# LemonATsu/UNet-PhaseGen

Measured on AMD Instinct MI355X. Metric: spectrogram-frames/sec (train fwd+bwd), higher is better.
Workload: dtype f32; 1 GPU; train.py full step (fwd + cos/sin/mag loss + bwd + Adam), UNetModel(1024, 2048), per-GPU batch 64 x 1024 bins x 256 frames (BASELINE configs[2]); global_batch=64, frames=256, channels=1024, parallelism=dp1, grad_allreduce_payload=fp32, adam=fused into the wgrad epilogues

## Files before the change

### include/phasegen.h

```cpp
#ifndef PHASEGEN_H
#define PHASEGEN_H
#include <stdint.h>

#ifdef __cplusplus
extern "C" {
#endif

#define PG_VERSION 400

enum { PG_OK = 0, PG_ERR_NULL = -1, PG_ERR_SHAPE = -2, PG_ERR_ALIGN = -3, PG_ERR_UNSUPPORTED = -4,
       PG_ERR_WORKSPACE = -5 };

enum { PG_ACT_NONE = 0, PG_ACT_LEAKY02 = 1 , PG_ACT_RELU = 2  };

struct pg_adam_args;
typedef struct pg_conv_args {
    int32_t B, Cin, Cout, Lin, Lout, k, stride, pad;
    const float* x;  int64_t x_bs;
    int32_t x_act;
    int32_t precision;
    const float* w;
    float* y;        int64_t y_bs;
    const float* dy; int64_t dy_bs;
    float* dx;       int64_t dx_bs;
    const float* dx_add; int64_t dx_add_bs;
    const float* dx_ref; int64_t dx_ref_bs;
    int32_t dx_mask;
    int32_t schedule;
    float* dw;
    int32_t y_act; int32_t y2_act;
    float* y2;       int64_t y2_bs;
    void* workspace; int64_t workspace_bytes;
    const struct pg_adam_args* adam;
} pg_conv_args;
int64_t pg_workspace_bytes_conv(void);
int64_t pg_workspace_bytes_wgrad(const pg_conv_args* a, int32_t op);
enum { PG_PREC_FP32 = 0, PG_PREC_BF16 = 1, PG_PREC_BF16X3 = 2 };
enum { PG_SCHED_AUTO = 0, PG_SCHED_TILE_PER_WG = 1, PG_SCHED_FORCE_STREAMK = 2, PG_SCHED_NO_RAW = 4, PG_SCHED_NO_TALL = 8,
       PG_SCHED_CONTENDED = 16, PG_SCHED_NO_PS = 128, PG_SCHED_NO_RAW3 = 0x2000, PG_SCHED_ALL_RAW3 = 0x4000, PG_SCHED_NO_COLSPLIT = 0x20000, PG_SCHED_COLSPLIT = 0x40000 };
#define PG_SCHED_OVERSUB(f) (((f) & 15) << 8)

int pg_conv1d_fwd(const pg_conv_args* a, void* stream);
int pg_conv1d_dgrad(const pg_conv_args* a, void* stream);
int pg_conv1d_wgrad(const pg_conv_args* a, void* stream);
int pg_convt1d_fwd(const pg_conv_args* a, void* stream);
int pg_convt1d_dgrad(const pg_conv_args* a, void* stream);
int pg_convt1d_wgrad(const pg_conv_args* a, void* stream);
enum { PG_OP_CONV1D_FWD = 0, PG_OP_CONV1D_DGRAD = 1, PG_OP_CONV1D_WGRAD = 2,
       PG_OP_CONVT1D_FWD = 3, PG_OP_CONVT1D_DGRAD = 4, PG_OP_CONVT1D_WGRAD = 5 };
int pg_conv_describe(const pg_conv_args* a, int32_t op, char* buf, int32_t buflen);

#define PG_H_HEAD 32
typedef struct pg_convh_args {
    int32_t B, Cin, Cout, Lin, Lout, k, stride, pad;
    int32_t transposed;
    int32_t schedule;
    const uint16_t* x; int64_t x_bs;
    int32_t x_pitch; int32_t _pad0;
    const uint16_t* w;
    float* y; int64_t y_bs;
    uint16_t* yh; int64_t yh_bs; int32_t yh_pitch; int32_t yh_act;
    uint16_t* yh2; int64_t yh2_bs; int32_t yh2_pitch; int32_t yh2_act;
    void* workspace; int64_t workspace_bytes;
} pg_convh_args;
int pg_conv_fwd_h(const pg_convh_args* a, void* stream);
int pg_conv_fwd_h_supported(const pg_convh_args* a);
int pg_conv_fwd_h_describe(const pg_convh_args* a, char* buf, int32_t buflen);
int64_t pg_shadow_elems(int32_t Cin, int32_t Cout, int32_t k, int32_t stride, int32_t transposed);
int pg_shadow_weights(const float* w, uint16_t* wh, int32_t Cin, int32_t Cout, int32_t k, int32_t stride, int32_t transposed, void* stream);
typedef struct pg_cast_args { int32_t B, C, L, pitch, act, _pad0; const float* x; int64_t x_bs; uint16_t* y; int64_t y_bs; } pg_cast_args;
int pg_cast_rows_bf16(const pg_cast_args* a, void* stream);

typedef struct pg_bn_args {
    int32_t B, C, L; float eps, momentum;
    const float* x;  int64_t x_bs;
    float* y;        int64_t y_bs;
    const float* gamma; const float* beta;
    float* save_mean; float* save_invstd;
    float* running_mean; float* running_var;
    const float* dy; int64_t dy_bs;
    float* dx;       int64_t dx_bs;
    float* dgamma; float* dbeta;
    int32_t y_act; int32_t y2_act;
    float* y2;       int64_t y2_bs;
    uint16_t* yh;  int64_t yh_bs;  int32_t yh_pitch;  int32_t yh_act;
    uint16_t* yh2; int64_t yh2_bs; int32_t yh2_pitch; int32_t yh2_act;
    int64_t* num_batches_tracked;
} pg_bn_args;
int pg_bn_fwd(const pg_bn_args* a, void* stream);
int pg_bn_bwd(const pg_bn_args* a, void* stream);

typedef struct pg_clipnorm_args {
// ... 144 lines not shown
```

### unet-phasegen_amd/csrc/conv_common.h

```cpp
#pragma once
#include <hip/hip_runtime.h>
#include <stdint.h>
#include "phasegen.h"
#include "pg_common.h"

namespace pgconv {

struct IgemmParams {
    const float* x; long x_bs;
    const float* w;
    const float* pt; long pt_bs;
    float* y; long y_bs;
    const float* add; long add_bs;
    const float* ref; long ref_bs;
    unsigned x_bytes, w_bytes, pt_bytes;
    int B, Q, M, Lx, Ly, k, s, p;
    int act_x, act_p, mask_mode;
    int U, u_off;
    int LP; float inv_LP;
    int a_vec;
    int tilesM, tilesN;
    int g_ps;
    int tn_stride;
    float* y2; long y2_bs; float y_slope, y2_slope;
    float* ws;
    int nslab;
    int whole;
    int sr;
    int n_lo;
    int x_pitch;
    unsigned short* yh; long yh_bs; int yh_pitch; float yh_slope;
    unsigned short* yh2; long yh2_bs; int yh2_pitch; float yh2_slope;
    float* ad_p; float* ad_m; float* ad_v; PgAdamScalars ad;
    const float* qk; unsigned qk_bytes; int qk_bs, Lq;
    const float* pk; unsigned pk_bytes; int Kp;
};

}
using pgconv::IgemmParams;

namespace {


constexpr int WMB = 4;
constexpr int BM = 64 * WMB, BN = 128, BK = 16, NT = 256;
constexpr int TILE_A = BM * BK, TILE_B = BN * BK;
constexpr int STAGE = TILE_A + TILE_B;
constexpr int AE = BM / 16;

typedef float f32x16 __attribute__((ext_vector_type(16)));


typedef __amdgpu_buffer_rsrc_t rsrc_t;
constexpr int OOB = 0x7ffffff0;
__device__ __forceinline__ rsrc_t make_rsrc(const float* p, unsigned bytes) {
    return __builtin_amdgcn_make_buffer_rsrc(const_cast<float*>(p), 0, (int)bytes, 0x00020000);
}
__device__ __forceinline__ float bload(rsrc_t r, int elem_off, bool ok) {
    return __builtin_bit_cast(float, __builtin_amdgcn_raw_buffer_load_b32(r, ok ? elem_off * 4 : OOB, 0, 0));
}

__device__ __forceinline__ int xcd_remap(int bid, int nwg) {
    const int xcd = bid & 7, local = bid >> 3, q = nwg >> 3, r = nwg & 7;
    return (xcd < r ? xcd * (q + 1) : r * (q + 1) + (xcd - r) * q) + local;
}

template <int MB, int NB> struct AccT { f32x16 c[MB][NB]; };
using Acc = AccT<WMB, 2>;
using AccR = AccT<2, 4>;

__device__ __forceinline__ int dma_kt(int lane, int w) { return ((((lane >> 2) & 3) ^ w) << 2) | (lane & 3); }
__device__ __forceinline__ int dma_row(int lane, int w, int e) { return 16 * e + 4 * w + (lane >> 4); }

__device__ __forceinline__ int dma16_row(int lane, int w, int e) { return (4 * e + w) * 16 + (lane >> 2); }
__device__ __forceinline__ int dma16_kc(int lane) { return ((lane & 3) ^ ((lane >> 4) & 3)) << 2; }
#ifndef PG_ABL
#define PG_ABL 0
#endif
#if PG_ABL == 4
#define PG_ADDR(x) ((x) & 0x3f0)
#else
#define PG_ADDR(x) (x)
#endif
__device__ __forceinline__ void dma16(rsrc_t r, float* lds_wave_uniform, int byte_off) {
    __builtin_amdgcn_raw_ptr_buffer_load_lds(r, lds_wave_uniform, 16, PG_ADDR(byte_off), 0, 0, 0);
}
__device__ __forceinline__ void dma4(rsrc_t r, float* lds_wave_uniform, int byte_off) {
    __builtin_amdgcn_raw_ptr_buffer_load_lds(r, lds_wave_uniform, 4, PG_ADDR(byte_off), 0, 0, 0);
// ... 325 lines not shown
#pragma unroll
        for (int i = 0; i < MB; ++i)
#pragma unroll
            for (int q = 0; q < 2; ++q) {
                const int mb = m0 + wm * (MB * 32) + i * 32 + 16 * q + 4 * (lane >> 5);
                float pp[8], mm[8], vv[8];
#pragma unroll
                for (int r = 0; r < 8; ++r) {
                    const int m = mb + (r & 3) + 8 * (r >> 2);
                    const unsigned o = (unsigned)(m < p.M ? m : 0) * (unsigned)Ntot + (unsigned)n;
                    pp[r] = p.ad_p[o]; mm[r] = p.ad_m[o]; vv[r] = p.ad_v[o];
                }
#pragma unroll
                for (int r = 0; r < 8; ++r) {
                    const int m = mb + (r & 3) + 8 * (r >> 2);
                    if (m >= p.M) continue;
                    const unsigned o = (unsigned)m * (unsigned)Ntot + (unsigned)n;
                    pg_adam_one(pp[r], acc.c[i][j][8 * q + r], mm[r], vv[r], p.ad.omb1, p.ad.b2, p.ad.omb2, p.ad.step_size, p.ad.bc2_sqrt,
                                p.ad.eps, p.ad.gs);
                    p.ad_p[o] = pp[r]; p.ad_m[o] = mm[r]; p.ad_v[o] = vv[r];
                }
                __builtin_amdgcn_sched_barrier(0);
            }
    }
}

constexpr int NEVER = 0x40000000;
constexpr int FAR = (int)0x80000000u;


#if PG_ABL == 7
#define PG_STAMP(i) { unsigned long long t_; asm volatile("s_memtime %0\n\ts_waitcnt lgkmcnt(0)" : "=s"(t_) :: "memory"); \
                      __builtin_amdgcn_sched_barrier(0); if (i) st_sum[i - 1] += t_ - st_prev; st_prev = t_; }
#define PG_STAMP_FLUSH if (lane == 0) { for (int i_ = 0; i_ < 3; ++i_) atomicAdd((unsigned long long*)p.ws + i_, st_sum[i_]); \
                                        atomicAdd((unsigned long long*)p.ws + 3, (unsigned long long)(se - sb)); }
#define PG_STAMP_DECL unsigned long long st_sum[3] = {0, 0, 0}, st_prev = 0;
#else
#define PG_STAMP(i)
#define PG_STAMP_FLUSH
#define PG_STAMP_DECL
#endif

__device__ __forceinline__ void divmod24(int n, int d, float inv, int& q, int& r) {
    q = (int)((float)n * inv);
    r = n - q * d;
    if (r < 0) { r += d; --q; }
    if (r >= d) { r -= d; ++q; }
}

constexpr int RBM = 128, RBN = 256;
constexpr int RS2 = 768, RS1 = 384;
constexpr int raw_gap(int tj) { return tj >= 8 ? 16 : tj; }
constexpr int RTILE_A = RBM * BK;
constexpr int g_wlp(int kw, int s) { return kw == 32 ? 64 : (kw == 8 ? (s == 1 ? 24 : 40) : 36); }

inline bool unet_ks(int k, int s) { return (k == 32 && s == 2) || (k == 8 && s == 1) || (k == 8 && s == 2) || (k == 4 && s == 2) || (k == 5 && s == 2); }

enum Kind { KIND_F, KIND_T, KIND_G };

}

namespace pgconv {
hipError_t launch_im2col(int kind, const IgemmParams& p, int grid, hipStream_t st, int prec);
hipError_t launch_raw_ft(int kind, const IgemmParams& p, int grid, hipStream_t st, int prec);
hipError_t launch_raw_ft_tall(int kind, const IgemmParams& p, int grid, hipStream_t st, int prec);
hipError_t launch_raw_g(const IgemmParams& p, int grid, hipStream_t st, int prec);
hipError_t launch_h3(int kind, const IgemmParams& p, int grid, hipStream_t st);
bool raw3_covers(int kind, const IgemmParams& p);
hipError_t launch_raw3(int kind, const IgemmParams& p, int grid, hipStream_t st);
bool h_supported(int kind, const IgemmParams& p);
}
```

### unet-phasegen_amd/csrc/conv_igemm.hip

```cpp
#include <hip/hip_runtime.h>
#include <cstring>
#include <cmath>
#include <algorithm>
#include "conv_fixup.h"

namespace {

constexpr int WG_PER_CU = 2;
constexpr int MAX_STREAMK_WG = 2048;
constexpr long WS_PER_WG = 2L * ACC_REGS * NT * 4;
constexpr long WS_STREAMK = (long)MAX_STREAMK_WG * WS_PER_WG;

struct Knobs {
    int prec;
    int force_mode;
    int no_raw;
    int no_tall;
    int oversub;
    int contended;
    int no_ps;
    int no_raw3;
    int all_raw3;
    int sr;
    int force_colsplit;
    int no_colsplit;
};
int decode_knobs(const pg_conv_args* a, Knobs& k) {
    if (a->precision < 0 || a->precision > 2) return pg_fail(PG_ERR_UNSUPPORTED, "conv: precision must be PG_PREC_FP32, PG_PREC_BF16 or PG_PREC_BF16X3");
    const int sc = a->schedule;
    if (sc < 0 || (sc & ~0x7ffff) || ((sc >> 17) & 3) == 3 || (sc & 3) == 3 || ((sc >> 8) & 15) > 8) return pg_fail(PG_ERR_SHAPE, "conv: bad schedule bits");
    k.prec = a->precision;
    k.force_mode = sc & 3; k.no_raw = (sc >> 2) & 1; k.no_tall = (sc >> 3) & 1;
    k.oversub = (sc >> 8) & 15; if (!k.oversub) k.oversub = 4;
    k.contended = (sc >> 4) & 1;
    if ((sc >> 5) & 3) return pg_fail(PG_ERR_UNSUPPORTED, "conv: schedule bits 5-6 (tile families removed in 0.4)");
    k.no_ps = (sc >> 7) & 1;
    k.no_raw3 = (sc >> 13) & 1;
    k.all_raw3 = (sc >> 14) & 1;
    k.sr = ((sc >> 15) & 3) ? 1 << (((sc >> 15) & 3) - 1) : 0;
    k.no_colsplit = (sc >> 17) & 1;
    k.force_colsplit = (sc >> 18) & 1;
    if (k.no_raw3 && k.all_raw3) return pg_fail(PG_ERR_SHAPE, "conv: schedule bits 13 and 14 exclude each other");
    return PG_OK;
}

bool fixup_wide(int grid, long split_tiles) { return split_tiles > 0 && grid >= 8 * split_tiles; }

int pick_grid(long tiles, int nslab, IgemmParams& p, long ws_bytes, const Knobs& kn, bool one_wave) {
    const long total = tiles * (long)nslab;
    const long slots = (long)pg_cu_count() * (one_wave ? 1 : WG_PER_CU), ws_per_wg = one_wave ? 2 * WS_PER_WG : WS_PER_WG;
    ws_bytes = std::min(ws_bytes, WS_STREAMK);
    p.whole = 0;
    if (kn.force_mode == 0 && !kn.contended && tiles % slots == 0) {
        if (tiles <= slots * kn.oversub) return (int)tiles;
        for (long mult = kn.oversub; mult >= 1; --mult)
            if (tiles % (slots * mult) == 0) return (int)(slots * mult);
    }
    long mult = total / (256 * slots);
    if (mult > kn.oversub) mult = kn.oversub;
    if (mult < 1) mult = 1;
    long G = slots * mult;
    if (G > MAX_STREAMK_WG) G = (MAX_STREAMK_WG / slots) * slots;
    if (G > total) G = total;
    const bool can = p.ws && ws_bytes >= G * ws_per_wg && total < 0x7fffffffL;
    if (kn.force_mode == 1 || !can) return (int)tiles;
    if (kn.force_mode == 2) return (int)G;
    if (!kn.contended && tiles > slots) {
        const long whole = tiles / slots * slots, rem = tiles - whole;
        if (rem * nslab >= slots * 8 && whole + slots <= MAX_STREAMK_WG && ws_bytes >= (whole + slots) * ws_per_wg) {
            p.whole = (int)whole;
            return (int)(whole + slots);
        }
    }
    return total >= slots * 8 ? (int)G : (int)tiles;
}

bool raw_supported(Kind kind, const IgemmParams& p, const Knobs& kn, int tn = RBN) {
    if (kn.no_raw || !unet_ks(p.k, p.s) || (kind == KIND_F && p.k == 5 && p.Q % 2)) return false;
    if (kind == KIND_G) return p.LP >= 16;
    const bool t = kind == KIND_T;
    const int kv = p.k == 5 ? 8 : p.k, kwp = t ? kv / p.s : kv, sc = t ? 1 : p.s, lcol = t ? p.U : p.Ly;
    const int tj = kwp < 16 ? kwp : 16;
    const int nseg_max = (lcol - 1 + tn - 1) / lcol + 1;
    return sc * (tn - 1) + tj + raw_gap(tj) * (nseg_max - 1) + (t ? tj : 0) <= (sc == 1 ? RS1 : RS2);
}

long g_pack_layout(IgemmParams& p) {
    const int cps = (p.LP + 15) / 16;
    const long gimax = p.g_ps ? 16L * (cps - 1) : (long)p.LP - 1;
    long lq = (long)p.s * gimax + g_wlp(p.k, p.s);
    if (lq < (long)p.p + p.Lx) lq = (long)p.p + p.Lx;
    lq = (lq + 3) / 4 * 4;
    const long kp = p.g_ps ? 16L * cps : 16L * p.nslab;
    const long qbytes = (long)p.B * p.Q * lq * 4, pbytes = (p.g_ps ? (long)p.B : 1L) * p.M * kp * 4;
// ... 127 lines not shown
struct ConvOp { Kind kind; bool tr, swap; const char* null_msg; };
const ConvOp CONV_OPS[6] = {
    {KIND_F, false, false, "conv1d_fwd: x, w, y required"},
    {KIND_T, false, true, "conv1d_dgrad: dy, w, dx required"},
    {KIND_G, false, false, "conv1d_wgrad: dy, x, dw required"},
    {KIND_T, true, false, "convt1d_fwd: x, w, y required"},
    {KIND_F, true, true, "convt1d_dgrad: dy, w, dx required"},
    {KIND_G, true, true, "convt1d_wgrad: dy, x, dw required"}};

int plan_conv(int op, const pg_conv_args* a, bool ptrs, ConvPlan& pl) {
    const ConvOp& o = CONV_OPS[op];
    if (int e = check_geom(a, o.tr)) return e;
    Knobs kn; if (int e = decode_knobs(a, kn)) return e;
    IgemmParams p = {};
    p.B = a->B; p.k = a->k; p.s = a->stride; p.p = a->pad;
    p.M = o.swap ? a->Cin : a->Cout; p.Q = o.swap ? a->Cout : a->Cin; p.Lx = o.swap ? a->Lout : a->Lin;
    const int lo = o.swap ? a->Lin : a->Lout;
    p.x = o.swap ? a->dy : a->x; p.x_bs = o.swap ? a->dy_bs : a->x_bs; p.act_x = o.swap ? PG_ACT_NONE : a->x_act;
    if (o.kind == KIND_G) {
        p.pt = o.swap ? a->x : a->dy; p.pt_bs = o.swap ? a->x_bs : a->dy_bs; p.act_p = o.swap ? a->x_act : PG_ACT_NONE;
        p.LP = lo; p.y = a->dw;
    } else if (o.swap) {
        p.w = a->w; p.Ly = lo; p.y = a->dx; p.y_bs = a->dx_bs; p.y_slope = 1.0f; p.y2_slope = 1.0f;
        p.add = a->dx_add; p.add_bs = a->dx_add_bs; p.ref = a->dx_ref; p.ref_bs = a->dx_ref_bs;
        p.mask_mode = a->dx_ref ? a->dx_mask : 0;
    } else {
        p.w = a->w; p.Ly = lo; p.y = a->y; p.y_bs = a->y_bs; p.y_slope = pg_act_slope(a->y_act);
        p.y2 = a->y2; p.y2_bs = a->y2_bs; p.y2_slope = pg_act_slope(a->y2_act);
    }
    if (ptrs && (!p.x || !p.y || !(o.kind == KIND_G ? p.pt : p.w))) return pg_fail(PG_ERR_NULL, o.null_msg);
    long rows = p.M, cols = (long)p.B * p.Ly, K = (long)p.Q * p.k;
    if (o.kind == KIND_T) {
        p.u_off = p.p / p.s;
        p.U = (p.Ly - 1 + p.p) / p.s - p.u_off + 1;
        if (p.U <= 0) return pg_fail(PG_ERR_SHAPE, "convT: empty output");
        rows = (long)p.M * p.s; cols = (long)p.B * p.U; K = (long)p.Q * ((p.k + p.s - 1) / p.s);
    } else if (o.kind == KIND_G) {
        cols = (long)p.Q * p.k; K = (long)p.B * p.LP;
    }
    if (int e = set_extents(p)) return e;
    if (int e = o.kind == KIND_G ? set_fused_adam(p, a) : PG_OK) return e;
    p.ws = (float*)a->workspace;
    pl.kind = o.kind; pl.prec = kn.prec; pl.pack = 0;
    pl.has_tail = split_columns(o.kind, p, kn, rows, cols, K, a->workspace_bytes);
    if (pl.has_tail) {
        const long full = cols / RBN * RBN;
        if (int e = plan_part(FAM_RAW3, o.kind, kn, p, rows, 0, full, K, a->workspace_bytes, pl.main)) return e;
        return plan_part(FAM_RAW_TALL, o.kind, kn, p, rows, full, cols, K, a->workspace_bytes, pl.tail);
    }
    const Family fam = pick_family(o.kind, p, kn, rows, cols);
    if (int e = plan_part(fam, o.kind, kn, p, rows, 0, cols, K, a->workspace_bytes, pl.main)) return e;
    if ((pl.main.fam == FAM_G_RAW || pl.main.fam == FAM_G_PS) && kn.prec == 0 && (pl.pack = g_pack_layout(pl.main.p)) < 0)
        return pg_fail(PG_ERR_SHAPE, "wgrad: packed operand exceeds 2 GiB (31-bit buffer offsets)");
    return PG_OK;
}

int h3_params(const pg_convh_args* a, bool ptrs, IgemmParams& p, Knobs& kn) {
    if (!a) return pg_fail(PG_ERR_NULL, "conv_fwd_h: null args");
    if (a->B <= 0 || a->Cin <= 0 || a->Cout <= 0 || a->Lin <= 0 || a->Lout <= 0 || a->k <= 0 || a->stride <= 0 || a->pad < 0)
        return pg_fail(PG_ERR_SHAPE, "conv_fwd_h: non-positive dimension");
    const bool tr = a->transposed != 0;
    const long lo = tr ? (long)(a->Lin - 1) * a->stride - 2L * a->pad + a->k : ((long)a->Lin + 2L * a->pad - a->k) / a->stride + 1;
    if (lo != a->Lout) return pg_fail(PG_ERR_SHAPE, "conv_fwd_h: Lout inconsistent with Lin/k/stride/pad");
    if (ptrs && (!a->x || !a->w || (!a->y && !a->yh && !a->yh2))) return pg_fail(PG_ERR_NULL, "conv_fwd_h: x, w and at least one output required");
    if (((uintptr_t)a->x & 3) || ((uintptr_t)a->w & 15) || (a->x_bs & 1) || (a->x_pitch & 1))
        return pg_fail(PG_ERR_ALIGN, "conv_fwd_h: x must be 4-byte aligned with even pitch / batch stride, w 16-byte aligned");
    if (a->x_pitch <= a->Lin) return pg_fail(PG_ERR_SHAPE, "conv_fwd_h: x_pitch must exceed Lin (zero tail of at least one element)");
    if ((a->yh && a->yh_pitch < a->Lout) || (a->yh2 && a->yh2_pitch < a->Lout)) return pg_fail(PG_ERR_SHAPE, "conv_fwd_h: output pitch below Lout");
    pg_conv_args kb = {};
    kb.schedule = a->schedule;
    if (int e = decode_knobs(&kb, kn)) return e;
    p = {};
    p.x = reinterpret_cast<const float*>(a->x); p.x_bs = a->x_bs; p.x_pitch = a->x_pitch;
    p.w = reinterpret_cast<const float*>(a->w);
    p.y = a->y; p.y_bs = a->y_bs; p.y_slope = 1.0f; p.y2_slope = 1.0f;
    p.yh = a->yh; p.yh_bs = a->yh_bs; p.yh_pitch = a->yh_pitch; p.yh_slope = pg_act_slope(a->yh_act);
    p.yh2 = a->yh2; p.yh2_bs = a->yh2_bs; p.yh2_pitch = a->yh2_pitch; p.yh2_slope = pg_act_slope(a->yh2_act);
    p.B = a->B; p.Q = a->Cin; p.M = a->Cout; p.Lx = a->Lin; p.Ly = a->Lout; p.k = a->k; p.s = a->stride; p.p = a->pad;
    p.ws = (float*)a->workspace;
    const long xe = ((long)(p.B - 1) * p.x_bs + (long)p.Q * p.x_pitch) * 2;
    if (xe <= 0 || xe >= 0x7ffffff0L) return pg_fail(PG_ERR_SHAPE, "conv_fwd_h: activation tensor exceeds 2 GiB (31-bit buffer offsets)");
    p.x_bytes = (unsigned)xe;
    const int kwp = tr ? pg_shadow_taps(p.k, p.s) : p.k;
    const long wbytes = (long)p.M * (tr ? p.s : 1) * p.Q * kwp * 2;
    if (wbytes >= 0x7ffffff0L) return pg_fail(PG_ERR_SHAPE, "conv_fwd_h: weight shadow exceeds 2 GiB");
    p.w_bytes = (unsigned)wbytes;
    if (tr) {
        p.u_off = p.p / p.s;
        p.U = (p.Ly - 1 + p.p) / p.s - p.u_off + 1;
        if (p.U <= 0) return pg_fail(PG_ERR_SHAPE, "conv_fwd_h: empty output");
    }
    if (!pgconv::h_supported(tr ? KIND_T : KIND_F, p)) return pg_fail(PG_ERR_UNSUPPORTED, "conv_fwd_h: geometry not covered by the bf16-resident kernels (use the fp32-tensor entry points)");
    return PG_OK;
}

int plan_h3(const pg_convh_args* a, ConvPlan& pl) {
    Knobs kn;
    ConvPart& c = pl.main;
    IgemmParams& p = c.p;
    if (int e = h3_params(a, true, p, kn)) return e;
    const bool tr = a->transposed != 0;
    pl.kind = tr ? KIND_T : KIND_F; pl.prec = 0; pl.has_tail = false; pl.pack = 0; c.fam = FAM_H3;
    const long rows = tr ? (long)p.M * p.s : p.M, cols = (long)p.B * (tr ? p.U : p.Ly);
    p.tilesM = (int)((rows + 255) / 256);
    p.tilesN = (int)((cols + 255) / 256);
    p.tn_stride = 256;
    p.nslab = (int)((long)p.Q * (tr ? pg_shadow_taps(p.k, p.s) : p.k) / 32);
    c.tiles = (long)p.tilesM * p.tilesN;
    if (c.tiles <= 0 || c.tiles > 0x0fffffffL || p.nslab <= 0) return pg_fail(PG_ERR_SHAPE, "conv_fwd_h: empty or oversize grid");
    set_grid(c, kn, a->workspace_bytes);
    return PG_OK;
}

hipError_t launch_fixup(const ConvPlan& pl, const ConvPart& c, hipStream_t st) {
    typedef void (*Fn)(const IgemmParams, int);
#define FIX2(KIND, MB, NB, WN) {conv_fixup_kernel<KIND, MB, NB, WN, false>, conv_fixup_kernel<KIND, MB, NB, WN, true>}
    static const Fn table[4][4][2] = {
        {FIX2(FIX_F, WMB, 2, 2), FIX2(FIX_T, WMB, 2, 2), FIX2(FIX_G, WMB, 2, 2), {}},
        {FIX2(FIX_F, 2, 4, 2), FIX2(FIX_T, 2, 4, 2), FIX2(FIX_G, 2, 4, 2), FIX2(FIX_T_PM, 2, 4, 2)},
        {FIX2(FIX_F, 2, 4, 1), FIX2(FIX_T, 2, 4, 1), {}, FIX2(FIX_T_PM, 2, 4, 1)},
        {FIX2(FIX_F, 8, 2, 4), FIX2(FIX_T, 8, 2, 4), {}, {conv_fixup_kernel<FIX_T_PM, 8, 2, 4, false>, nullptr}}};
#undef FIX2
    const int geom = c.fam == FAM_IM2COL ? 0 : (c.fam == FAM_RAW_TALL ? 2 : (c.fam == FAM_RAW3 || c.fam == FAM_H3 ? 3 : 1));
    const bool pm = pl.kind == KIND_T && c.p.s == 2 && (c.fam == FAM_RAW || c.fam == FAM_RAW_TALL || c.fam == FAM_RAW3);
    const bool wide = c.fixup == FIXUP_WIDE;
    const Fn fn = table[geom][pm ? FIX_T_PM : (int)pl.kind][wide];
    if (!fn) return hipErrorInvalidDeviceFunction;
    const long blocks = (c.tiles - c.p.whole) * (geom == 3 ? 16 : 8) * (wide ? 4 : 1);
    hipLaunchKernelGGL(fn, dim3((unsigned)blocks), dim3(NT), 0, st, c.p, c.grid);
    return hipGetLastError();
}

hipError_t part_kernel(const ConvPlan& pl, const ConvPart& c, hipStream_t st, char* name = nullptr) {
    const IgemmParams& p = c.p;
    const Kind kind = pl.kind;
    const char* tk = kind == KIND_T ? "true" : "false";
    hipError_t e = hipSuccess;
    switch (c.fam) {
        case FAM_RAW_TALL:
            if (name) snprintf(name, 96, "conv_raw_kernel<%d, %d, %s, %d, 1>", p.k, p.s, tk, pl.prec);
            else e = pgconv::launch_raw_ft_tall(kind, p, c.grid, st, pl.prec);
            break;
        case FAM_RAW:
            if (name) snprintf(name, 96, "conv_raw_kernel<%d, %d, %s, %d, 2>", p.k, p.s, tk, pl.prec);
            else e = pgconv::launch_raw_ft(kind, p, c.grid, st, pl.prec);
            break;
        case FAM_G_RAW:
        case FAM_G_PS:
            if (name) snprintf(name, 96, "conv_g_%s_kernel<%d, %d, %d>", c.fam == FAM_G_PS ? "ps" : "raw", p.k, p.s, pl.prec);
            else e = pgconv::launch_raw_g(p, c.grid, st, pl.prec);
            break;
        case FAM_IM2COL:
            if (name) snprintf(name, 96, "conv_%c_kernel<0, 0, %d>", "ftg"[kind], pl.prec);
            else e = pgconv::launch_im2col(kind, p, c.grid, st, pl.prec);
            break;
        case FAM_RAW3:
            if (name) snprintf(name, 96, "conv_raw3_kernel<%d, %d, %s, %s>", p.k, p.s, tk, p.act_x == PG_ACT_NONE ? "false" : "true");
            else e = pgconv::launch_raw3(kind, p, c.grid, st);
            break;
        case FAM_H3:
            if (name) snprintf(name, 96, "conv_h3_kernel<%d, %d, %s>", kind == KIND_T && p.k == 5 ? 8 : p.k, p.s, tk);
            else e = pgconv::launch_h3(kind, p, c.grid, st);
            break;
    }
    if (!name && e == hipSuccess && c.fixup != FIXUP_NONE) e = launch_fixup(pl, c, st);
    return e;
}

void describe(const ConvPlan& pl, char* buf, int buflen) {
    static const char* const fixup_name[] = {"none", "plain", "wide"};
    const ConvPart& c = pl.main;
    char name[96];
    (void)part_kernel(pl, c, nullptr, name);
    snprintf(buf, (size_t)buflen, "%s|grid=%d|tiles=%ld|slabs=%d|split=%d|whole=%d|fixup=%s", name, c.grid, c.tiles, c.p.nslab,
             (int)(c.fixup != FIXUP_NONE), c.p.whole, fixup_name[c.fixup]);
    if (!pl.has_tail) return;
    (void)part_kernel(pl, pl.tail, nullptr, name);
    const size_t n = strlen(buf);
    if (n + 7 < (size_t)buflen) snprintf(buf + n, (size_t)buflen - n, "|tail=%s,grid=%d", name, pl.tail.grid);
}

int execute(ConvPlan& pl, long ws_bytes, hipStream_t st) {
    IgemmParams& p = pl.main.p;
    if (pl.pack) {
        if (!p.ws || ws_bytes < WS_STREAMK + pl.pack)
            return pg_fail(PG_ERR_WORKSPACE, "wgrad: the fp32 kernels need pg_workspace_bytes_wgrad() bytes of workspace (packed operands)");
        p.qk = reinterpret_cast<const float*>(reinterpret_cast<char*>(p.ws) + WS_STREAMK);
        p.pk = reinterpret_cast<const float*>(reinterpret_cast<const char*>(p.qk) + ((long)p.qk_bytes + 255) / 256 * 256);
    }
    hipError_t e = part_kernel(pl, pl.main, st);
    if (e == hipSuccess && pl.has_tail) e = part_kernel(pl, pl.tail, st);
    return e == hipSuccess ? PG_OK : pg_fail((int)e, hipGetErrorString(e));
}

int run_conv(int op, const pg_conv_args* a, void* stream) {
    ConvPlan pl;
    if (int e = plan_conv(op, a, true, pl)) return e;
    return execute(pl, a->workspace_bytes, (hipStream_t)stream);
}

}

// ... 44 lines not shown
```

### unet-phasegen_amd/csrc/conv_raw_wgrad.hip

```cpp
#include "conv_common.h"

namespace {

template <int KW, int S> struct GRaw {
    static constexpr int WL = 15 * S + KW;
    static constexpr int WLP = g_wlp(KW, S);
    static constexpr int NQT = RBN / KW;
    static constexpr int TNV = NQT * KW;
    static constexpr int SUB = NQT * WLP;
    static constexpr int SUBS = (SUB + 63) / 64 * 64;
    static constexpr int NE = (SUB + NT - 1) / NT;
    static constexpr int STG = RTILE_A + 2 * SUBS;
    static constexpr int SUBP = (SUB + 255) / 256 * 256;
    static_assert(WL <= WLP, "window does not fit its slot");
};

template <int KW, int S, int BF>
__device__ __forceinline__ void g_raw_bf(const IgemmParams& p) {
    using C = GRaw<KW, S>;
    __shared__ __attribute__((aligned(16))) float lds[2 * C::STG];
    const int tid = threadIdx.x, lane = tid & 63;
    const int wv = __builtin_amdgcn_readfirstlane(tid >> 6), wm = wv >> 1, wn = wv & 1;
    const int kt = dma_kt(lane, wv);
    const rsrc_t rp = make_rsrc(p.pt, p.pt_bytes), rx = make_rsrc(p.x, p.x_bytes);
// ... 519 lines not shown

        int gb = sb / cps, gc = sb - gb * cps;
#define GPF_ISSUE(STAGE_PTR)                                                                              \
    {   const int gbc = min(gb, p.B - 1), gi = gc << 4;                                                   \
        _Pragma("unroll") for (int e = 0; e < 2; ++e) dma16s(rp, (STAGE_PTR) + wv * 256 + e * 1024, pv[e], gbc * pbs4 + gi * 4); \
        const int sw_ = gbc * qbs4 + S * gi * 4;                                                          \
        _Pragma("unroll") for (int e = 0; e < NE16; ++e)                                                  \
            if (4 * (e * NT + wv * 64) < C::SUB) dma16s(rx, (STAGE_PTR) + RTILE_A + 4 * (e * NT + wv * 64), woff[e], sw_); \
        if (++gc == cps) { gc = 0; ++gb; }                                                                \
    }
        GPF_ISSUE(lds)
        __syncthreads();
        for (int sl = sb; sl < se; ++sl) {
            const int cur = (sl - sb) & 1;
            GPF_ISSUE(lds + (cur ^ 1) * STG)
            __builtin_amdgcn_sched_barrier(0);
            {
                const float* As = lds + cur * STG;
                const float* Bw = As + RTILE_A;
                const int r = lane & 31, h = lane >> 5, sw = (r >> 2) & 3;
                const float* ap = As + (wm * 64 + r) * BK;
                f32x4 a[2][2];
                float b[4][8];
#pragma unroll
                for (int i = 0; i < 2; ++i) a[i][0] = *reinterpret_cast<const f32x4*>(ap + i * 32 * BK + (((2 * h) ^ sw) << 2));
#pragma unroll
                for (int ip = 0; ip < 4; ++ip) {
                    if (ip == 2) {
#pragma unroll
                        for (int i = 0; i < 2; ++i) a[i][1] = *reinterpret_cast<const f32x4*>(ap + i * 32 * BK + (((2 * h + 1) ^ sw) << 2));
                    }
#pragma unroll
                    for (int jb = 0; jb < 4; ++jb) { b[jb][2 * ip] = Bw[bbase[jb] + S * 2 * ip]; b[jb][2 * ip + 1] = Bw[bbase[jb] + S * (2 * ip + 1)]; }
                }
#pragma unroll
                for (int kk = 0; kk < 8; ++kk)
#pragma unroll
                    for (int i = 0; i < 2; ++i)
#pragma unroll
                        for (int j = 0; j < 4; ++j)
                            acc.c[i][j] = __builtin_amdgcn_mfma_f32_32x32x2f32(a[i][kk >> 2][kk & 3], b[j][kk], acc.c[i][j], 0, 0, 0);
            }
            __builtin_amdgcn_sched_barrier(0);
            __syncthreads();
        }
#undef GPF_ISSUE
        if (sb == 0 && se == p.nslab) epilogue_g<S, 2, 4>(p, acc, m0, n0, lane, wm, wn, n0 + C::TNV);
        else store_partial(p.ws, g, slot, acc, tid);
        pos += se - sb;
        slot = 1;
    }
}

template <int KW, int S, int BF>
__global__ __launch_bounds__(NT, 2) void conv_g_raw_kernel(const IgemmParams p) {
    if constexpr (BF == 0) g_raw_f32<KW, S>(p);
    else g_raw_bf<KW, S, BF>(p);
}
template <int KW, int S, int BF>
__global__ __launch_bounds__(NT, 2) void conv_g_ps_kernel(const IgemmParams p) {
    if constexpr (BF == 0) g_ps_f32<KW, S>(p);
    else g_ps_bf<KW, S, BF>(p);
}

__global__ __launch_bounds__(256) void pack_rows_kernel(const float* __restrict__ src, long bs, int C, int L, int F, int W, unsigned n,
                                                       float slope, float* __restrict__ dst) {
    for (unsigned i = blockIdx.x * 256u + threadIdx.x; i < n; i += gridDim.x * 256u) {
        const unsigned r = i / (unsigned)W, b = r / (unsigned)C, c = r - b * (unsigned)C;
        const int t = (int)(i - r * (unsigned)W) - F;
        float v = 0.f;
        if ((unsigned)t < (unsigned)L) {
            v = src[(long)b * bs + (long)c * L + t];
            if (slope != 1.0f) v = pg_act_apply(v, slope);
        }
        dst[i] = v;
    }
}
__global__ __launch_bounds__(256) void pack_flat_kernel(const float* __restrict__ src, long bs, int B, int LP, int Kp, unsigned n,
                                                       float slope, float* __restrict__ dst) {
    for (unsigned i = blockIdx.x * 256u + threadIdx.x; i < n; i += gridDim.x * 256u) {
        const unsigned m = i / (unsigned)Kp, k = i - m * (unsigned)Kp, b = k / (unsigned)LP, t = k - b * (unsigned)LP;
        float v = 0.f;
        if ((int)b < B) {
            v = src[(long)b * bs + (long)m * LP + t];
            if (slope != 1.0f) v = pg_act_apply(v, slope);
        }
        dst[i] = v;
    }
}
unsigned pack_grid(unsigned n) { return (n + 255u) / 256u < 2048u ? (n + 255u) / 256u : 2048u; }

hipError_t pack_g(const IgemmParams& p, hipStream_t st) {
    float* const qk = const_cast<float*>(p.qk);
    float* const pk = const_cast<float*>(p.pk);
    const unsigned nq = (unsigned)(p.qk_bytes / 4), np = (unsigned)(p.pk_bytes / 4);
    hipLaunchKernelGGL(pack_rows_kernel, dim3(pack_grid(nq)), dim3(256), 0, st, p.x, p.x_bs, p.Q, p.Lx, p.p, p.Lq, nq, pg_act_slope(p.act_x), qk);
    if (p.g_ps) hipLaunchKernelGGL(pack_rows_kernel, dim3(pack_grid(np)), dim3(256), 0, st, p.pt, p.pt_bs, p.M, p.LP, 0, p.Kp, np, pg_act_slope(p.act_p), pk);
    else hipLaunchKernelGGL(pack_flat_kernel, dim3(pack_grid(np)), dim3(256), 0, st, p.pt, p.pt_bs, p.B, p.LP, p.Kp, np, pg_act_slope(p.act_p), pk);
    return hipGetLastError();
}

template <int KW, int S>
hipError_t launch_g_raw(const IgemmParams& p, int grid, hipStream_t st, int prec) {
    if (prec == 0) {
        if (hipError_t e = pack_g(p, st)) return e;
    }
    if (p.g_ps) {
        if (prec == 1) hipLaunchKernelGGL((conv_g_ps_kernel<KW, S, 1>), dim3(grid), dim3(NT), 0, st, p);
        else if (prec == 2) hipLaunchKernelGGL((conv_g_ps_kernel<KW, S, 2>), dim3(grid), dim3(NT), 0, st, p);
        else hipLaunchKernelGGL((conv_g_ps_kernel<KW, S, 0>), dim3(grid), dim3(NT), 0, st, p);
        return hipGetLastError();
    }
    if (prec == 1) hipLaunchKernelGGL((conv_g_raw_kernel<KW, S, 1>), dim3(grid), dim3(NT), 0, st, p);
    else if (prec == 2) hipLaunchKernelGGL((conv_g_raw_kernel<KW, S, 2>), dim3(grid), dim3(NT), 0, st, p);
    else hipLaunchKernelGGL((conv_g_raw_kernel<KW, S, 0>), dim3(grid), dim3(NT), 0, st, p);
    return hipGetLastError();
}

}

hipError_t pgconv::launch_raw_g(const IgemmParams& p, int grid, hipStream_t st, int prec) {
    if (p.k == 32) return launch_g_raw<32, 2>(p, grid, st, prec);
    if (p.k == 8 && p.s == 1) return launch_g_raw<8, 1>(p, grid, st, prec);
    if (p.k == 8) return launch_g_raw<8, 2>(p, grid, st, prec);
    if (p.k == 5) return launch_g_raw<5, 2>(p, grid, st, prec);
    return launch_g_raw<4, 2>(p, grid, st, prec);
}
```

### unet-phasegen_amd/phasegen/ops.py

```python
import contextlib
import ctypes as C
import threading

import torch

from . import _lib
from ._lib import ACT_LEAKY, ACT_NONE, ACT_RELU, SCHED_CONTENDED, SCHED_TILE_PER_WG


def _stream():
    return C.c_void_p(torch.cuda.current_stream().cuda_stream)


def _on_current_device(t, name):
    if t.device.index != torch.cuda.current_device():
        raise ValueError(f"{name}: tensor is on {t.device} but the current device is cuda:{torch.cuda.current_device()} "
                         "(wrap the call in torch.cuda.device(...))")


class KernelTimer:

    def __init__(self):
        self.records = {}
        self.plans = {}
# ... 104 lines not shown
        return buf

    def clear(self):
        self.d.clear()


_conv_ws = _StreamCache()
_caches = [_conv_ws]


def _workspace(cache, device, need, what):
    if need < 0:
        _lib.check(int(need), what)
    ws = cache.get(device, lambda: need, need)
    return ws.data_ptr(), ws.numel()


def conv_workspace(device):
    return _conv_ws.get(device, _lib.load().pg_workspace_bytes_conv)


def release_workspaces():
    for c in _caches:
        c.clear()


_PRECISIONS = {"fp32": 0, "f32": 0, "bf16": 1, "bf16x3": 2, 0: 0, 1: 1, 2: 2}


class _Defaults(threading.local):
    precision = 0
    schedule = 0
    stft_single = 0


_tls = _Defaults()


def precision_code(mode):
    if mode not in _PRECISIONS:
        raise ValueError(f"conv precision {mode!r}: expected fp32 / bf16 / bf16x3 (or 0 / 1 / 2)")
    return _PRECISIONS[mode]


def set_conv_precision(mode):
    _tls.precision = precision_code(mode)


def current_schedule():
    return _tls.schedule


def set_conv_schedule(mode):
    if mode < 0 or (mode & ~0x7e0ff) or (mode & 0x60000) == 0x60000 or (mode & 3) == 3 or (mode & 0x70) or (mode & 0x6000) == 0x6000:
        raise ValueError("conv schedule: bad mode")
    _tls.schedule = (_tls.schedule & 0xf00) | mode


def set_conv_oversubscribe(factor):
    if not 1 <= factor <= 8:
        raise ValueError("conv oversubscribe: factor must be 1..8")
    _tls.schedule = (_tls.schedule & ~0xf00) | (factor << 8)


def set_stft_mode(single_frame):
    _tls.stft_single = int(bool(single_frame))


@contextlib.contextmanager
def conv_options(precision=None, schedule=None):
    old = (_tls.precision, _tls.schedule)
    if precision is not None:
        _tls.precision = precision_code(precision)
    if schedule is not None:
        _tls.schedule = schedule
    try:
        yield
    finally:
        _tls.precision, _tls.schedule = old


def _conv_args(transposed, B, Cin, Cout, Lin, k, s, p, device=None, precision=None, schedule=None):
    a = _lib.ConvArgs()
    a.precision = _tls.precision if precision is None else precision_code(precision)
    a.schedule = _tls.schedule if schedule is None else schedule
    a.B, a.Cin, a.Cout, a.Lin, a.k, a.stride, a.pad = B, Cin, Cout, Lin, k, s, p
    a.Lout = convt_out_len(Lin, k, s, p) if transposed else conv_out_len(Lin, k, s, p)
    if device is not None:
        ws = conv_workspace(device)
        a.workspace, a.workspace_bytes = ws.data_ptr(), ws.numel()
    return a


def _geom(transposed, w_shape):
    a, b, k = w_shape
    return (a, b, k) if transposed else (b, a, k)


def conv_fwd(x, w, y, stride, pad, x_act=ACT_NONE, transposed=False, y_act=ACT_NONE, y2=None, y2_act=ACT_NONE,
             precision=None, schedule=None):
    Cin, Cout, k = _geom(transposed, w.shape)
    B, _, Lin = x.shape
    a = _conv_args(transposed, B, Cin, Cout, Lin, k, stride, pad, x.device, precision, schedule)
    if tuple(x.shape) != (B, Cin, Lin) or tuple(y.shape) != (B, Cout, a.Lout):
        raise ValueError(f"conv_fwd: shapes x{tuple(x.shape)} w{tuple(w.shape)} y{tuple(y.shape)} inconsistent (Lout {a.Lout})")
    a.x, a.x_bs = _act3(x, "x")
    a.y, a.y_bs = _act3(y, "y")
# ... 699 lines not shown
```

Measured before the change: 98590 frames/s.

## Add direct-register A-operand fp32 wgrad kernels for selected conv families

Result: no change. 98570 frames/s (median of 4 runs) (-0.0%).

```diff
diff --git a/include/phasegen.h b/include/phasegen.h
--- a/include/phasegen.h
+++ b/include/phasegen.h
@@ -37,7 +37,8 @@
 int64_t pg_workspace_bytes_wgrad(const pg_conv_args* a, int32_t op);
 enum { PG_PREC_FP32 = 0, PG_PREC_BF16 = 1, PG_PREC_BF16X3 = 2 };
 enum { PG_SCHED_AUTO = 0, PG_SCHED_TILE_PER_WG = 1, PG_SCHED_FORCE_STREAMK = 2, PG_SCHED_NO_RAW = 4, PG_SCHED_NO_TALL = 8,
-       PG_SCHED_CONTENDED = 16, PG_SCHED_NO_PS = 128, PG_SCHED_NO_RAW3 = 0x2000, PG_SCHED_ALL_RAW3 = 0x4000, PG_SCHED_NO_COLSPLIT = 0x20000, PG_SCHED_COLSPLIT = 0x40000 };
+       PG_SCHED_CONTENDED = 16, PG_SCHED_NO_PS = 128, PG_SCHED_NO_RAW3 = 0x2000, PG_SCHED_ALL_RAW3 = 0x4000, PG_SCHED_NO_COLSPLIT = 0x20000, PG_SCHED_COLSPLIT = 0x40000,
+       PG_SCHED_G_ALT = 0x80000 };
 #define PG_SCHED_OVERSUB(f) (((f) & 15) << 8)
 
 int pg_conv1d_fwd(const pg_conv_args* a, void* stream);
diff --git a/unet-phasegen_amd/csrc/conv_common.h b/unet-phasegen_amd/csrc/conv_common.h
--- a/unet-phasegen_amd/csrc/conv_common.h
+++ b/unet-phasegen_amd/csrc/conv_common.h
@@ -34,6 +34,7 @@
     float* ad_p; float* ad_m; float* ad_v; PgAdamScalars ad;
     const float* qk; unsigned qk_bytes; int qk_bs, Lq;
     const float* pk; unsigned pk_bytes; int Kp;
+    int g_direct;
 };
 
 }
@@ -465,6 +466,7 @@
 constexpr int RS2 = 768, RS1 = 384;
 constexpr int raw_gap(int tj) { return tj >= 8 ? 16 : tj; }
 constexpr int RTILE_A = RBM * BK;
+constexpr bool g_direct_family(int kw, int s, bool per_sample) { return per_sample ? (kw == 8 && s == 1) || kw == 5 : kw == 32; }
 constexpr int g_wlp(int kw, int s) { return kw == 32 ? 64 : (kw == 8 ? (s == 1 ? 24 : 40) : 36); }
 
 inline bool unet_ks(int k, int s) { return (k == 32 && s == 2) || (k == 8 && s == 1) || (k == 8 && s == 2) || (k == 4 && s == 2) || (k == 5 && s == 2); }
diff --git a/unet-phasegen_amd/csrc/conv_igemm.hip b/unet-phasegen_amd/csrc/conv_igemm.hip
--- a/unet-phasegen_amd/csrc/conv_igemm.hip
+++ b/unet-phasegen_amd/csrc/conv_igemm.hip
@@ -24,11 +24,12 @@
     int sr;
     int force_colsplit;
     int no_colsplit;
+    int g_alt;
 };
 int decode_knobs(const pg_conv_args* a, Knobs& k) {
     if (a->precision < 0 || a->precision > 2) return pg_fail(PG_ERR_UNSUPPORTED, "conv: precision must be PG_PREC_FP32, PG_PREC_BF16 or PG_PREC_BF16X3");
     const int sc = a->schedule;
-    if (sc < 0 || (sc & ~0x7ffff) || ((sc >> 17) & 3) == 3 || (sc & 3) == 3 || ((sc >> 8) & 15) > 8) return pg_fail(PG_ERR_SHAPE, "conv: bad schedule bits");
+    if (sc < 0 || (sc & ~0xfffff) || ((sc >> 17) & 3) == 3 || (sc & 3) == 3 || ((sc >> 8) & 15) > 8) return pg_fail(PG_ERR_SHAPE, "conv: bad schedule bits");
     k.prec = a->precision;
     k.force_mode = sc & 3; k.no_raw = (sc >> 2) & 1; k.no_tall = (sc >> 3) & 1;
     k.oversub = (sc >> 8) & 15; if (!k.oversub) k.oversub = 4;
@@ -40,6 +41,7 @@
     k.sr = ((sc >> 15) & 3) ? 1 << (((sc >> 15) & 3) - 1) : 0;
     k.no_colsplit = (sc >> 17) & 1;
     k.force_colsplit = (sc >> 18) & 1;
+    k.g_alt = (sc >> 19) & 1;
     if (k.no_raw3 && k.all_raw3) return pg_fail(PG_ERR_SHAPE, "conv: schedule bits 13 and 14 exclude each other");
     return PG_OK;
 }
@@ -273,6 +275,8 @@
     if (int e = plan_part(fam, o.kind, kn, p, rows, 0, cols, K, a->workspace_bytes, pl.main)) return e;
     if ((pl.main.fam == FAM_G_RAW || pl.main.fam == FAM_G_PS) && kn.prec == 0 && (pl.pack = g_pack_layout(pl.main.p)) < 0)
         return pg_fail(PG_ERR_SHAPE, "wgrad: packed operand exceeds 2 GiB (31-bit buffer offsets)");
+    IgemmParams& pm = pl.main.p;
+    pm.g_direct = pl.pack > 0 && ((g_direct_family(pm.k, pm.s, pm.g_ps != 0) && !pm.ad_p) != (kn.g_alt != 0));
     return PG_OK;
 }
 
@@ -368,7 +372,7 @@
             break;
         case FAM_G_RAW:
         case FAM_G_PS:
-            if (name) snprintf(name, 96, "conv_g_%s_kernel<%d, %d, %d>", c.fam == FAM_G_PS ? "ps" : "raw", p.k, p.s, pl.prec);
+            if (name) snprintf(name, 96, "conv_g_%s_kernel<%d, %d, %d>", c.fam == FAM_G_PS ? "ps" : "raw", p.k, p.s, p.g_direct ? 3 : pl.prec);
             else e = pgconv::launch_raw_g(p, c.grid, st, pl.prec);
             break;
         case FAM_IM2COL:
diff --git a/unet-phasegen_amd/csrc/conv_raw_wgrad.hip b/unet-phasegen_amd/csrc/conv_raw_wgrad.hip
--- a/unet-phasegen_amd/csrc/conv_raw_wgrad.hip
+++ b/unet-phasegen_amd/csrc/conv_raw_wgrad.hip
@@ -595,14 +595,219 @@
     }
 }
 
+__device__ __forceinline__ f32x4 bload16s(rsrc_t r, int lane_off, int uniform_off) {
+    return __builtin_bit_cast(f32x4, __builtin_amdgcn_raw_buffer_load_b128(r, lane_off, uniform_off, 0));
+}
+__device__ __forceinline__ void a_direct_offsets(const IgemmParams& p, int m0, int wm, int lane, int (&av)[2]) {
+#pragma unroll
+    for (int i = 0; i < 2; ++i) {
+        const int m = m0 + wm * 64 + i * 32 + (lane & 31);
+        av[i] = m < p.M ? (m * p.Kp + 8 * (lane >> 5)) * 4 : FAR;
+    }
+}
+#define GD_READ_B(B, Bw)                                                                                   \
+    _Pragma("unroll") for (int ip = 0; ip < 4; ++ip)                                                       \
+        _Pragma("unroll") for (int jb = 0; jb < 4; ++jb) {                                                 \
+            B[jb][2 * ip] = (Bw)[bbase[jb] + S * 2 * ip]; B[jb][2 * ip + 1] = (Bw)[bbase[jb] + S * (2 * ip + 1)]; }
+#define GD_MFMA(A, B)                                                                                      \
+    _Pragma("unroll") for (int kk = 0; kk < 8; ++kk)                                                       \
+        _Pragma("unroll") for (int i = 0; i < 2; ++i)                                                      \
+            _Pragma("unroll") for (int j = 0; j < 4; ++j)                                                  \
+                acc.c[i][j] = __builtin_amdgcn_mfma_f32_32x32x2f32(A[i][kk >> 2][kk & 3], B[j][kk], acc.c[i][j], 0, 0, 0);
+
+template <int KW, int S>
+__device__ __forceinline__ void g_raw_f32d(const IgemmParams& p) {
+    using C = GRaw<KW, S>;
+    constexpr int NP = 2 * C::SUBP / 4;
+    constexpr int NE2 = (NP + NT - 1) / NT;
+    constexpr int STG = 2 * C::SUBP;
+    static_assert(C::WLP % 4 == 0, "16-byte window pieces");
+    __shared__ __attribute__((aligned(16))) float lds[2 * STG];
+    const int tid = threadIdx.x, lane = tid & 63;
+    const int wv = __builtin_amdgcn_readfirstlane(tid >> 6), wm = wv >> 1, wn = wv & 1;
+    const rsrc_t rp = make_rsrc(p.pk, p.pk_bytes), rx = make_rsrc(p.qk, p.qk_bytes);
+    const int qbs4 = p.qk_bs * 4, klast4 = (p.nslab - 1) * BK * 4;
+    Walk wk(p);
+    while (wk.more()) {
+        int tile, sb, se;
+        wk.segment(p, tile, sb, se);
+        const int m0 = (tile / p.tilesN) * RBM, n0 = (tile % p.tilesN) * C::TNV;
+        const int qbase = (tile % p.tilesN) * C::NQT;
+        int av[2], woff[NE2];
+        a_direct_offsets(p, m0, wm, lane, av);
+#pragma unroll
+        for (int e = 0; e < NE2; ++e) {
+            const int pc = tid + NT * e, sub = pc >= C::SUBP / 4 ? 1 : 0, f = 4 * pc - sub * C::SUBP, ql = f / C::WLP, v0 = f - ql * C::WLP;
+            woff[e] = (f < C::SUB && qbase + ql < p.Q) ? ((qbase + ql) * p.Lq + v0) * 4 : FAR;
+        }
+        int bbase[4];
+#pragma unroll
+        for (int jb = 0; jb < 4; ++jb) {
+            const int c = wn * 128 + jb * 32 + (lane & 31), qc = c / KW;
+            bbase[jb] = qc * C::WLP + (c - qc * KW) + S * 8 * (lane >> 5);
+        }
+        AccR acc;
+#pragma unroll
+        for (int i = 0; i < 2; ++i)
+#pragma unroll
+            for (int j = 0; j < 4; ++j)
+#pragma unroll
+                for (int r = 0; r < 16; ++r) acc.c[i][j][r] = 0.f;
+
+        int gb, gi;
+        { const int k0 = sb * BK; gb = k0 / p.LP; gi = k0 - gb * p.LP; }
+        int kc_cur, kc_next;
+#define GRD_ISSUE(STAGE_PTR, AN, K0)                                                                      \
+    {   const int sa = min((K0) * 4, klast4);                                                             \
+        const int kc = p.LP - gi;                                                                         \
+        const int sw0 = min(gb, p.B - 1) * qbs4 + S * gi * 4;                                             \
+        const int sw1 = (kc < 16 && gb + 1 < p.B) ? (gb + 1) * qbs4 : sw0;                                \
+        _Pragma("unroll") for (int e = 0; e < NE2; ++e) {                                                 \
+            const int pc0 = e * NT + wv * 64;                                 \
+            if ((e + 1) * NT <= NP || pc0 < NP)                                                           \
+                dma16s(rx, (STAGE_PTR) + 4 * pc0, woff[e], pc0 >= C::SUBP / 4 ? sw1 : sw0);               \
+        }                                                                                                 \
+        _Pragma("unroll") for (int c = 0; c < 2; ++c)                                                     \
+            _Pragma("unroll") for (int i = 0; i < 2; ++i) AN[i][c] = bload16s(rp, av[i] + 16 * c, sa);    \
+        kc_next = kc < 16 ? kc : 16;                                                                      \
+        gi += BK; if (gi >= p.LP) { gi -= p.LP; ++gb; }                                                   \
+    }
+#define GRD_STEP(A, AN, CUR, NXT)                                                                         \
+    {   PG_STAMP(0)                                                                                       \
+        GRD_ISSUE(NXT, AN, (sl + 1) * BK)                                                                 \
+        __builtin_amdgcn_sched_barrier(0);                                                                \
+        PG_STAMP(1)                                                                                       \
+        {   const float* Bw = (CUR);                                                                      \
+            float b[4][8];                                                                                \
+            if (kc_cur >= 16) {                                                                           \
+                GD_READ_B(b, Bw)                                                                          \
+            } else {        \
+                typedef const volatile __attribute__((address_space(3))) float* lds_vptr;                 \
+                const lds_vptr Bv = (lds_vptr)Bw;                                                         \
+                const int shift = C::SUBP - S * kc_cur;                                                   \
+                _Pragma("unroll") for (int i = 0; i < 8; ++i) {                                           \
+                    const int d = (8 * (lane >> 5) + i >= kc_cur) ? shift : 0;                            \
+                    _Pragma("unroll") for (int jb = 0; jb < 4; ++jb) b[jb][i] = Bv[bbase[jb] + S * i + d]; \
+                }                                                                                         \
+            }                                                                                             \
+            GD_MFMA(A, b)                                                                                 \
+        }                                                                                                 \
+        __builtin_amdgcn_sched_barrier(0);                                                                \
+        PG_STAMP(2)                                                                                       \
+        kc_cur = kc_next;                                                                                 \
+        __syncthreads();                                                                                  \
+        PG_STAMP(3)                                                                                       \
+    }
+        PG_STAMP_DECL
+        f32x4 a0[2][2], a1[2][2];
+        GRD_ISSUE(lds, a0, sb * BK)
+        kc_cur = kc_next;
+        __syncthreads();
+        for (int sl = sb;;) {
+            GRD_STEP(a0, a1, lds, lds + STG)
+            if (++sl == se) break;
+            GRD_STEP(a1, a0, lds + STG, lds)
+            if (++sl == se) break;
+        }
+        PG_STAMP_FLUSH
+#undef GRD_STEP
+#undef GRD_ISSUE
+        if (sb == 0 && se == p.nslab) epilogue_g<S, 2, 4>(p, acc, m0, n0, lane, wm, wn, n0 + C::TNV);
+        else store_partial(p.ws, wk.g, wk.slot, acc, tid);
+        wk.next(se - sb);
+    }
+}
+
+template <int KW, int S>
+__device__ __forceinline__ void g_ps_f32d(const IgemmParams& p) {
+    using C = GRaw<KW, S>;
+    constexpr int STG = (C::SUB + 255) / 256 * 256;
+    constexpr int NE16 = (C::SUB / 4 + NT - 1) / NT;
+    static_assert(C::WLP % 4 == 0, "16-byte window pieces");
+    __shared__ __attribute__((aligned(16))) float lds[2 * STG];
+    const int tid = threadIdx.x, lane = tid & 63;
+    const int wv = __builtin_amdgcn_readfirstlane(tid >> 6), wm = wv >> 1, wn = wv & 1;
+    const rsrc_t rp = make_rsrc(p.pk, p.pk_bytes), rx = make_rsrc(p.qk, p.qk_bytes);
+    const int pbs4 = p.M * p.Kp * 4, qbs4 = p.qk_bs * 4;
+    const int cps = p.Kp >> 4;
+    Walk wk(p);
+    while (wk.more()) {
+        int tile, sb, se;
+        wk.segment(p, tile, sb, se);
+        const int m0 = (tile / p.tilesN) * RBM, n0 = (tile % p.tilesN) * C::TNV;
+        const int qbase = (tile % p.tilesN) * C::NQT;
+        int av[2], woff[NE16];
+        a_direct_offsets(p, m0, wm, lane, av);
+#pragma unroll
+        for (int e = 0; e < NE16; ++e) {
+            const int f = 4 * (tid + NT * e), ql = f / C::WLP, v0 = f - ql * C::WLP;
+            woff[e] = (f < C::SUB && qbase + ql < p.Q) ? ((qbase + ql) * p.Lq + v0) * 4 : FAR;
+        }
+        int bbase[4];
+#pragma unroll
+        for (int jb = 0; jb < 4; ++jb) {
+            const int c = wn * 128 + jb * 32 + (lane & 31), qc = c / KW;
+            bbase[jb] = qc * C::WLP + (c - qc * KW) + S * 8 * (lane >> 5);
+        }
+        AccR acc;
+#pragma unroll
+        for (int i = 0; i < 2; ++i)
+#pragma unroll
+            for (int j = 0; j < 4; ++j)
+#pragma unroll
+                for (int r = 0; r < 16; ++r) acc.c[i][j][r] = 0.f;
+
+        int gb = sb / cps, gc = sb - gb * cps;
+#define GPD_ISSUE(STAGE_PTR, AN)                                                                          \
+    {   const int gbc = min(gb, p.B - 1), gi = gc << 4;                                                   \
+        const int sw_ = gbc * qbs4 + S * gi * 4, sa = gbc * pbs4 + gi * 4;                                \
+        _Pragma("unroll") for (int e = 0; e < NE16; ++e)                                                  \
+            if (4 * (e * NT + wv * 64) < C::SUB) dma16s(rx, (STAGE_PTR) + 4 * (e * NT + wv * 64), woff[e], sw_); \
+        _Pragma("unroll") for (int c = 0; c < 2; ++c)                                                     \
+            _Pragma("unroll") for (int i = 0; i < 2; ++i) AN[i][c] = bload16s(rp, av[i] + 16 * c, sa);    \
+        if (++gc == cps) { gc = 0; ++gb; }                                                                \
+    }
+#define GPD_STEP(A, AN, CUR, NXT)                                                                         \
+    {   GPD_ISSUE(NXT, AN)                                                                                \
+        __builtin_amdgcn_sched_barrier(0);                                                                \
+        {   const float* Bw = (CUR);                                                                      \
+            float b[4][8];                                                                                \
+            GD_READ_B(b, Bw)                                                                              \
+            GD_MFMA(A, b)                                                                                 \
+        }                                                                                                 \
+        __builtin_amdgcn_sched_barrier(0);                                                                \
+        __syncthreads();                                                                                  \
+    }
+        f32x4 a0[2][2], a1[2][2];
+        GPD_ISSUE(lds, a0)
+        __syncthreads();
+        for (int sl = sb;;) {
+            GPD_STEP(a0, a1, lds, lds + STG)
+            if (++sl == se) break;
+            GPD_STEP(a1, a0, lds + STG, lds)
+            if (++sl == se) break;
+        }
+#undef GPD_STEP
+#undef GPD_ISSUE
+        if (sb == 0 && se == p.nslab) epilogue_g<S, 2, 4>(p, acc, m0, n0, lane, wm, wn, n0 + C::TNV);
+        else store_partial(p.ws, wk.g, wk.slot, acc, tid);
+        wk.next(se - sb);
+    }
+}
+#undef GD_READ_B
+#undef GD_MFMA
+
+constexpr int BF_DIRECT = 3;
 template <int KW, int S, int BF>
 __global__ __launch_bounds__(NT, 2) void conv_g_raw_kernel(const IgemmParams p) {
     if constexpr (BF == 0) g_raw_f32<KW, S>(p);
+    else if constexpr (BF == BF_DIRECT) g_raw_f32d<KW, S>(p);
     else g_raw_bf<KW, S, BF>(p);
 }
 template <int KW, int S, int BF>
 __global__ __launch_bounds__(NT, 2) void conv_g_ps_kernel(const IgemmParams p) {
     if constexpr (BF == 0) g_ps_f32<KW, S>(p);
+    else if constexpr (BF == BF_DIRECT) g_ps_f32d<KW, S>(p);
     else g_ps_bf<KW, S, BF>(p);
 }
 
@@ -651,11 +856,13 @@
     if (p.g_ps) {
         if (prec == 1) hipLaunchKernelGGL((conv_g_ps_kernel<KW, S, 1>), dim3(grid), dim3(NT), 0, st, p);
         else if (prec == 2) hipLaunchKernelGGL((conv_g_ps_kernel<KW, S, 2>), dim3(grid), dim3(NT), 0, st, p);
+        else if (p.g_direct) hipLaunchKernelGGL((conv_g_ps_kernel<KW, S, BF_DIRECT>), dim3(grid), dim3(NT), 0, st, p);
         else hipLaunchKernelGGL((conv_g_ps_kernel<KW, S, 0>), dim3(grid), dim3(NT), 0, st, p);
         return hipGetLastError();
     }
     if (prec == 1) hipLaunchKernelGGL((conv_g_raw_kernel<KW, S, 1>), dim3(grid), dim3(NT), 0, st, p);
     else if (prec == 2) hipLaunchKernelGGL((conv_g_raw_kernel<KW, S, 2>), dim3(grid), dim3(NT), 0, st, p);
+    else if (p.g_direct) hipLaunchKernelGGL((conv_g_raw_kernel<KW, S, BF_DIRECT>), dim3(grid), dim3(NT), 0, st, p);
     else hipLaunchKernelGGL((conv_g_raw_kernel<KW, S, 0>), dim3(grid), dim3(NT), 0, st, p);
     return hipGetLastError();
 }
diff --git a/unet-phasegen_amd/phasegen/ops.py b/unet-phasegen_amd/phasegen/ops.py
--- a/unet-phasegen_amd/phasegen/ops.py
+++ b/unet-phasegen_amd/phasegen/ops.py
@@ -180,7 +180,7 @@
 
 
 def set_conv_schedule(mode):
-    if mode < 0 or (mode & ~0x7e0ff) or (mode & 0x60000) == 0x60000 or (mode & 3) == 3 or (mode & 0x70) or (mode & 0x6000) == 0x6000:
+    if mode < 0 or (mode & ~0xfe0ff) or (mode & 0x60000) == 0x60000 or (mode & 3) == 3 or (mode & 0x70) or (mode & 0x6000) == 0x6000:
         raise ValueError("conv schedule: bad mode")
     _tls.schedule = (_tls.schedule & 0xf00) | mode
 
```
